# svenstaro/bvh

Measured on NVIDIA H100. Metric: traversal_Mrays_per_s, higher is better.
Workload: dtype f32

## Files before the change

bvh_b200/csrc/capi.cu:

```cuda
#include "internal.h"
#include <cstdarg>
#include <cstring>
#include <vector>
#include <new>
#include <algorithm>
#include <cctype>
#include <sched.h>

namespace bvhb200 {

static thread_local std::string g_last_error;

void set_error(const char* fmt, ...) {
    char buf[1024];
    va_list ap;
    va_start(ap, fmt);
    vsnprintf(buf, sizeof(buf), fmt, ap);
    va_end(ap);
    g_last_error = buf;
}

int dalloc(bvhgpu_ctx* ctx, void** p, size_t bytes) {
    *p = nullptr;
    if (bytes == 0) bytes = 16;
// ... 912 lines not shown
        return rc;
    }
    return BVHGPU_OK;
}
BVH_EXPORT uint64_t bvhgpu_launch_count(const bvhgpu_ctx* ctx) { return ctx ? ctx->launches : 0; }
BVH_EXPORT int bvhgpu_set_option(bvhgpu_ctx* ctx, const char* name, int64_t value) {
    if (!ctx || !name) { set_error("set_option: null argument"); return BVHGPU_ERR_INVALID; }
    if (!strcmp(name, "traverse_slots")) { ctx->traverse_slots = value; return BVHGPU_OK; }
    if (!strcmp(name, "profile")) { ctx->profile = value; return BVHGPU_OK; }
    if (!strcmp(name, "build_small")) { ctx->build_small = value; return BVHGPU_OK; }
    if (!strcmp(name, "build_gang")) { ctx->build_gang = value; return BVHGPU_OK; }
    if (!strcmp(name, "build_subtree")) { ctx->build_subtree = value; return BVHGPU_OK; }
    if (!strcmp(name, "traverse_persistent")) { ctx->traverse_persistent = value; return BVHGPU_OK; }
    if (!strcmp(name, "traverse_stream")) { ctx->traverse_stream = value; return BVHGPU_OK; }
    if (!strcmp(name, "traverse_top")) { ctx->traverse_top = value; return BVHGPU_OK; }
    if (!strcmp(name, "walk_grid")) { ctx->walk_grid = value <= 0 ? 0 : (int)value; ctx->walk_grid_forced = value > 0; return BVHGPU_OK; }
    set_error("set_option: unknown option '%s'", name);
    return BVHGPU_ERR_INVALID;
}

BVH_EXPORT int bvhgpu_get_metric(bvhgpu_ctx* ctx, const char* name, double* out) {
    if (!ctx || !name || !out) { set_error("get_metric: null argument"); return BVHGPU_ERR_INVALID; }
    cudaEvent_t* ev = nullptr;
    if (!strncmp(name, "e2e_host_us_", 12) && name[12] >= '0' && name[12] <= '7' && !name[13]) { *out = ctx->host_us[name[12] - '0']; return BVHGPU_OK; }
    if (!strcmp(name, "stream_write_value")) { *out = (double)ctx->wv_ok; return BVHGPU_OK; }
    if (!strcmp(name, "host_streamed")) { *out = (double)ctx->last_streamed; return BVHGPU_OK; }
    if (!strcmp(name, "numa_node")) { *out = (double)ctx->numa_node; return BVHGPU_OK; }
    if (!strcmp(name, "walk_ms") && ctx->have_walk) ev = ctx->ev_walk;
    else if (!strcmp(name, "build_ms") && ctx->have_build) ev = ctx->ev_build;
    if (!ev && ctx->have_e2e && !strncmp(name, "e2e_", 4)) {
// ... 317 lines not shown
```

bvh_b200/csrc/common.cuh:

```cuda
#pragma once
#include <cuda_runtime.h>
#include <stdint.h>
#include <stddef.h>
#include "../../include/bvh_b200.h"

#define BVH_INVALID 0xFFFFFFFFu

namespace bvhb200 {

template <class T> struct Traits;

struct __align__(16) DAabbF { float min[3]; uint32_t pad0; float max[3]; uint32_t pad1; };
struct __align__(16) DAabbD { double min[3]; double max[3]; };

struct __align__(16) TNodeF { float min[3]; uint32_t skip; float max[3]; uint32_t shape; };
struct __align__(16) TNodeD { double min[3]; double max[3]; uint32_t skip; uint32_t shape; uint32_t pad[2]; };

template <> struct Traits<float> {
    using Aabb = bvh_aabb3f; using Ray = bvh_ray3f; using Node = bvh_node3f; using Flat = bvh_flat3f;
    using DAabb = DAabbF; using TNode = TNodeF;
    using Key = uint32_t;
    static constexpr Key KEY_POS_INF = 0xFF800000u;
    static constexpr Key KEY_NEG_INF = 0x007FFFFFu;
    __host__ __device__ static inline float eps() { return 1.1920928955078125e-7f; }
// ... 43 lines not shown

__device__ __forceinline__ float min_t(float a, float b) { return fminf(a, b); }
__device__ __forceinline__ float max_t(float a, float b) { return fmaxf(a, b); }
__device__ __forceinline__ double min_t(double a, double b) { return fmin(a, b); }
__device__ __forceinline__ double max_t(double a, double b) { return fmax(a, b); }

__device__ __forceinline__ float mul_rn(float a, float b) { return __fmul_rn(a, b); }
__device__ __forceinline__ float add_rn(float a, float b) { return __fadd_rn(a, b); }
__device__ __forceinline__ float sub_rn(float a, float b) { return __fsub_rn(a, b); }
__device__ __forceinline__ float div_rn(float a, float b) { return __fdiv_rn(a, b); }
__device__ __forceinline__ double mul_rn(double a, double b) { return __dmul_rn(a, b); }
__device__ __forceinline__ double add_rn(double a, double b) { return __dadd_rn(a, b); }
__device__ __forceinline__ double sub_rn(double a, double b) { return __dsub_rn(a, b); }
__device__ __forceinline__ double div_rn(double a, double b) { return __ddiv_rn(a, b); }

template <class T> __device__ __forceinline__ T center1(T mn, T mx) { return add_rn(mul_rn(mn, T(0.5)), mul_rn(mx, T(0.5))); }
template <class T> __device__ __forceinline__ T surface_area(const T mn[3], const T mx[3]) {
    const T sx = sub_rn(mx[0], mn[0]), sy = sub_rn(mx[1], mn[1]), sz = sub_rn(mx[2], mn[2]);
    return mul_rn(T(2), add_rn(add_rn(mul_rn(sx, sx), mul_rn(sy, sy)), mul_rn(sz, sz)));
}

template <int D, class T>
__device__ __forceinline__ bool slab_slice(const T o[D], const T inv[D], const T mn[D], const T mx[D], T& tmin_out, T& tmax_out) {
    T l[D], r[D];
#pragma unroll
    for (int k = 0; k < D; ++k) { l[k] = mul_rn(sub_rn(mn[k], o[k]), inv[k]); r[k] = mul_rn(sub_rn(mx[k], o[k]), inv[k]); }
    bool nan = (l[0] != l[0]) | (r[0] != r[0]);
#pragma unroll
    for (int k = 1; k < D; ++k) nan = nan | (l[k] != l[k]) | (r[k] != r[k]);
    T tmin = min_t(l[0], r[0]), tmax = max_t(l[0], r[0]);
// ... 66 lines not shown
```

bvh_b200/csrc/flatten.cu:

```cuda
#include "internal.h"
#include "update.cuh"

namespace bvhb200 {

template <class T>
__global__ void __launch_bounds__(256) flat_kernel(const typename Traits<T>::Node* __restrict__ nodes,
                                                   const uint32_t* __restrict__ node_start, uint32_t n_nodes,
                                                   typename Traits<T>::Flat* __restrict__ flat, const BuildStatus* __restrict__ status) {
    using Tr = Traits<T>;
    const uint32_t i = blockIdx.x * blockDim.x + threadIdx.x;
    if (i >= n_nodes) return;
    if (status->error | status->nan_found) return;
    const uint4 meta = *reinterpret_cast<const uint4*>(nodes + i);
    const bool leaf = meta.y == BVH_INVALID;
    if (i == 0) {
        if (leaf) {
            typename Tr::Flat f;
            for (int k = 0; k < 3; ++k) { f.aabb.min[k] = Tr::inf(); f.aabb.max[k] = -Tr::inf(); }
            f.entry_index = BVH_INVALID; f.exit_index = 1; f.shape_index = meta.w;
            flat[0] = f;
        }
        return;
    }
    const uint32_t nav = (i - 1) + node_start[i];
// ... 54 lines not shown
template <class T> int build_traversal_records(Tree<T>* tree) {
    bvhgpu_ctx* ctx = tree->ctx;
    if (tree->n == 0) { tree->n_trec = 0; return BVHGPU_OK; }
    const uint32_t n_trec = tree->n == 1 ? 1u : tree->n_nodes - 1;
    if (!tree->d_tnodes) BVH_TRY(dalloc_t(ctx, &tree->d_tnodes, n_trec));
    tree->n_trec = n_trec;
    tree->top_valid = false;
    trec_kernel<T><<<(tree->n_nodes + 255) / 256, 256, 0, ctx->stream>>>(tree->d_nodes, tree->n_nodes, tree->dims == 2 && tree->d_aabb_trav ? tree->d_aabb_trav : tree->d_aabb, tree->d_tnodes, tree->d_status, tree->dims);
    ctx->launches++;
    BVH_CUDA_TRY(cudaGetLastError());
    return BVHGPU_OK;
}

constexpr uint32_t TOP_BINS = 256;
__device__ __forceinline__ uint32_t top_bin(uint32_t c) { const uint32_t k = 31 - __clz(c); return 8 * k + (((c << 3) >> k) & 7u); }
__global__ void __launch_bounds__(256) top_hist_kernel(const bvh_node3f* __restrict__ nodes, uint32_t n_nodes, uint32_t* __restrict__ hist) {
    __shared__ uint32_t sh[TOP_BINS];
    sh[threadIdx.x] = 0;
    __syncthreads();
    const uint32_t i = blockIdx.x * blockDim.x + threadIdx.x;
    if (i >= 1 && i < n_nodes) atomicAdd(sh + top_bin(nodes[nodes[i].parent].shape), 1u);
    __syncthreads();
    if (sh[threadIdx.x]) atomicAdd(hist + threadIdx.x, sh[threadIdx.x]);
}
__global__ void __launch_bounds__(32) top_choose_kernel(const uint32_t* __restrict__ hist, uint32_t budget, uint32_t* __restrict__ hdr) {
    const uint32_t l = threadIdx.x & 31u, FULL = 0xffffffffu;
    uint32_t h[8], t = 0;
#pragma unroll
    for (int k = 0; k < 8; ++k) { h[k] = hist[8 * l + k]; t += h[k]; }
    uint32_t incl = t;
#pragma unroll
    for (int o = 1; o < 32; o <<= 1) { const uint32_t v = __shfl_down_sync(FULL, incl, o); if (l + o < 32) incl += v; }
    uint32_t run = incl - t, taken = 0, total = 0;
#pragma unroll
    for (int k = 7; k >= 0; --k) { run += h[k]; if (run <= budget) { ++taken; total = run; } }
    taken = __reduce_add_sync(FULL, taken);
    total = __reduce_max_sync(FULL, total);
    if (l) return;
    uint32_t C = 2;
    if (taken == 0) C = 0xFFFFFFFFu;
    else if (taken < TOP_BINS) { const uint32_t nb = TOP_BINS - taken, k = nb >> 3, sub = nb & 7u; C = (uint32_t)((((unsigned long long)(8 + sub) << k) + 7ull) >> 3); }
    hdr[0] = total; hdr[1] = C; hdr[2] = 0; hdr[3] = 0;
}
__global__ void __launch_bounds__(256) top_flag_kernel(const bvh_node3f* __restrict__ nodes, uint32_t n_nodes, const uint32_t* __restrict__ hdr, uint32_t* __restrict__ flags) {
    const uint32_t i = blockIdx.x * blockDim.x + threadIdx.x;
    if (i > n_nodes) return;
    const uint32_t C = hdr[1];
    uint32_t f = 0;
    if (i >= 1 && i < n_nodes) f = nodes[nodes[i].parent].shape >= C ? 1u : 0u;
    flags[i] = f;
}
__global__ void __launch_bounds__(256) top_emit_kernel(const bvh_node3f* __restrict__ nodes, uint32_t n_nodes, const TNodeF* __restrict__ trec,
                                                       const uint32_t* __restrict__ flags, const uint32_t* __restrict__ pre, float4* __restrict__ top) {
    const uint32_t i = blockIdx.x * blockDim.x + threadIdx.x;
    if (i == 0 || i >= n_nodes || !flags[i]) return;
    const uint32_t n_top = reinterpret_cast<const uint32_t*>(top)[0], C = reinterpret_cast<const uint32_t*>(top)[1];
    float4* lo = top + 2;
    float4* hi = lo + n_top;
    const uint32_t k = pre[i];
    if (k >= n_top) return;
    const uint4 meta = *reinterpret_cast<const uint4*>(nodes + i);
    const bool leaf = meta.y == BVH_INVALID;
    const uint32_t cnt = leaf ? 1u : meta.w;
    const TNodeF r = trec[i - 1];
    uint32_t w3, w7;
    if (!leaf && cnt >= C) { const uint32_t end = i + 2 * cnt - 1; w3 = pre[end < n_nodes ? end : n_nodes]; w7 = 0xFFFFFFFFu; }
    else if (leaf)         { w3 = k + 1; w7 = meta.w; }
    else                   { w3 = r.skip; w7 = 0x80000000u | i; }
    lo[k] = make_float4(r.min[0], r.min[1], r.min[2], __uint_as_float(w3));
    hi[k] = make_float4(r.max[0], r.max[1], r.max[2], __uint_as_float(w7));
}
}
#include <cub/device/device_scan.cuh>
namespace bvhb200 {
int build_top_records(Tree<float>* tree, uint32_t budget) {
    bvhgpu_ctx* ctx = tree->ctx;
    cudaStream_t st = ctx->stream;
    const uint32_t nn = tree->n_nodes;
    Scratch scratch(ctx);
    uint32_t *hist = nullptr, *flags = nullptr, *pre = nullptr;
    BVH_TRY(scratch.get(&hist, TOP_BINS));
    BVH_TRY(scratch.get(&flags, (size_t)nn + 1));
    BVH_TRY(scratch.get(&pre, (size_t)nn + 1));
    if (tree->d_top && tree->top_cap < budget) { dfree(ctx, tree->d_top); tree->d_top = nullptr; }
    if (!tree->d_top) { BVH_TRY(dalloc(ctx, &tree->d_top, 32 * ((size_t)budget + 1))); tree->top_cap = budget; }
    BVH_CUDA_TRY(cudaMemsetAsync(hist, 0, TOP_BINS * sizeof(uint32_t), st));
    const unsigned g = (nn + 256) / 256;
    uint32_t* hdr = reinterpret_cast<uint32_t*>(tree->d_top);
    top_hist_kernel<<<g, 256, 0, st>>>(tree->d_nodes, nn, hist);
    top_choose_kernel<<<1, 32, 0, st>>>(hist, budget, hdr);
    top_flag_kernel<<<g, 256, 0, st>>>(tree->d_nodes, nn, hdr, flags);
    size_t tmp_bytes = 0;
    cub::DeviceScan::ExclusiveSum(nullptr, tmp_bytes, flags, pre, (int)(nn + 1), st);
    unsigned char* tmp = nullptr;
    BVH_TRY(scratch.get(&tmp, tmp_bytes));
    cub::DeviceScan::ExclusiveSum(tmp, tmp_bytes, flags, pre, (int)(nn + 1), st);
    top_emit_kernel<<<g, 256, 0, st>>>(tree->d_nodes, nn, tree->d_tnodes, flags, pre, reinterpret_cast<float4*>(tree->d_top));
    ctx->launches += 5;
    BVH_CUDA_TRY(cudaGetLastError());
    tree->top_valid = true; tree->top_budget = budget;
    return BVHGPU_OK;
}

template <class T> int build_flat(Tree<T>* tree) {
    bvhgpu_ctx* ctx = tree->ctx;
    tree->n_flat = tree->n == 0 ? 0 : (tree->n == 1 ? 1 : 3 * (size_t)tree->n - 2);
    tree->have_flat = true;
    if (tree->n == 0) return BVHGPU_OK;
    if (!tree->d_flat) BVH_TRY(dalloc_t(ctx, &tree->d_flat, tree->n_flat));
    flat_kernel<T><<<(tree->n_nodes + 255) / 256, 256, 0, ctx->stream>>>(tree->d_nodes, tree->d_node_start, tree->n_nodes, tree->d_flat, tree->d_status);
    ctx->launches++;
    BVH_CUDA_TRY(cudaGetLastError());
    return BVHGPU_OK;
}

// ... 323 lines not shown
```

bvh_b200/csrc/internal.h:

```cpp
#pragma once
#include <cuda_runtime.h>
#include <string>
#include <cstdio>
#include "common.cuh"

namespace bvhb200 {

void set_error(const char* fmt, ...);

#define BVH_CUDA_TRY(expr)                                                                          \
    do {                                                                                            \
        cudaError_t _e = (expr);                                                                    \
        if (_e != cudaSuccess) {                                                                    \
            ::bvhb200::set_error("%s failed: %s (%s:%d)", #expr, cudaGetErrorString(_e), __FILE__, __LINE__); \
            return BVHGPU_ERR_CUDA;                                                                 \
        }                                                                                           \
    } while (0)

#define BVH_TRY(expr)                  \
    do {                               \
        int _s = (expr);               \
        if (_s != BVHGPU_OK) return _s; \
    } while (0)

// ... 26 lines not shown
    int64_t profile = 0;
    cudaEvent_t ev_walk[2] = {nullptr, nullptr};
    cudaEvent_t ev_build[2] = {nullptr, nullptr};
    bool have_walk = false, have_build = false;
    cudaStream_t copy_stream = nullptr, d2h_stream = nullptr;
    cudaEvent_t ev_order = nullptr, ev_total = nullptr;
    cudaEvent_t ev_chunk[16] = {}, ev_emit[16] = {};
    cudaEvent_t ev_e2e[5] = {};
    bool have_e2e = false;
    int stream_ok = -1;
    double host_us[8] = {0, 0, 0, 0, 0, 0, 0, 0};
    uint64_t slot_budget_words = 0;
    int last_streamed = -1;
    int64_t traverse_stream = -1;
    int64_t traverse_top = -1;
    uint32_t* d_ready = nullptr;
    int wv_ok = -1;
    uint32_t* d_async_err = nullptr;
    int numa_node = -1;
};
#define BVH_MAX_CHUNKS 16u

namespace bvhb200 {

template <class T> struct Tree {
    using Tr = Traits<T>;
    bvhgpu_ctx* ctx = nullptr;
    uint32_t n = 0;
    uint32_t n_nodes = 0;
    int dims = 3;
    typename Tr::DAabb* d_aabb = nullptr;
    typename Tr::DAabb* d_aabb_trav = nullptr;
    typename Tr::Node* d_nodes = nullptr;
    uint32_t* d_node_index = nullptr;
    uint32_t* d_node_start = nullptr;
    typename Tr::TNode* d_tnodes = nullptr;
    uint32_t n_trec = 0;
    void* d_top = nullptr;
    uint32_t top_cap = 0, top_budget = 0;
    bool top_valid = false;
    uint32_t* d_arrive = nullptr;
    uint8_t* d_bad = nullptr;
    void* d_sa_base = nullptr;
    void* d_tris = nullptr;
    typename Tr::Flat* d_flat = nullptr;
    size_t n_flat = 0;
    bool have_flat = false;
    BuildStatus* d_status = nullptr;
    BuildStatus* h_status = nullptr;
    bool status_pending = false;
    int failed_status = 0;
    std::string failed_message;
    uint32_t* d_offsets = nullptr; size_t offsets_cap = 0;
    uint32_t* d_hits = nullptr;    size_t hits_cap = 0;
    size_t last_total = 0, last_nrays = 0;
// ... 26 lines not shown
template <class T> int convert_aabbs(bvhgpu_ctx* ctx, const typename Traits<T>::Aabb* in_aabbs, uint32_t n,
                                     typename Traits<T>::DAabb* out, uint32_t* d_nan_flag);

struct BuildCtl;
template <class T> struct QSlot;
template <class T> struct TreeletSession { void* params = nullptr; QSlot<T>* q = nullptr; uint32_t* qseq = nullptr; uint32_t qmask = 0; BuildCtl* ctl = nullptr; };
template <class T> int treelet_begin(bvhgpu_ctx* ctx, Tree<T>* tree, uint32_t* sorted_ids, TreeletSession<T>* S);
template <class T> int treelet_finish(bvhgpu_ctx* ctx, Tree<T>* tree, TreeletSession<T>* S);

template <class T> int rebuild_subtrees(bvhgpu_ctx* ctx, Tree<T>* tree, const uint32_t* d_roots, const uint32_t* d_n_roots, const T* cb, uint32_t* idx0, bool cb_by_root);

template <class T> int build_lbvh(bvhgpu_ctx* ctx, const typename Traits<T>::Aabb* in_aabbs, uint32_t n, Tree<T>* tree, bool treelets);

template <class T> int build_traversal_records(Tree<T>* tree);
template <class T> int build_flat(Tree<T>* tree);
int build_top_records(Tree<float>* tree, uint32_t budget);
template <class T> int sah_cost(Tree<T>* tree, double* out2);
template <class T> int refit(Tree<T>* tree);
template <class T> int optimize(Tree<T>* tree, double max_growth);
template <class T> int update_changed(Tree<T>* tree, const uint32_t* d_changed, const typename Traits<T>::Aabb* d_fresh, uint32_t m, uint32_t* d_flags);
template <class T> int update_incremental(Tree<T>* tree, const uint32_t* d_changed, uint32_t m, double max_growth);
template <class T> int update_scatter(Tree<T>* tree, const uint32_t* d_changed, const typename Traits<T>::Aabb* d_fresh, uint32_t m);
template <class T> int ensure_sa_base(Tree<T>* tree);
template <class T> int rebuild_degraded(Tree<T>* tree, const uint32_t* d_dirty, uint32_t* d_cnts );

template <class T> int add_shapes(Tree<T>* tree, typename Traits<T>::DAabb* aabb_all, uint32_t k, double max_growth);
template <class T> int remove_shapes(Tree<T>* tree, const uint32_t* d_rm, uint32_t k);
int remove_check(bvhgpu_ctx* ctx, const uint32_t* d_idx, uint32_t k, uint32_t n, uint32_t* d_rm, uint32_t* d_flags);

template <class T> int traverse_device(Tree<T>* tree, int mode, const void* d_rays, uint32_t fmt,
                                       size_t nrays, uint32_t* d_offsets, uint32_t* d_hits, size_t cap, size_t* total,
// ... 40 lines not shown
```

bvh_b200/csrc/traverse.cu:

```cuda
#include "internal.h"
#include "csr.cuh"
#include "queries.cuh"
#include <cstdlib>
#include <cstring>
#include <algorithm>
#include <chrono>

namespace bvhb200 {

static inline uint32_t pick_slots(bvhgpu_ctx* ctx, uint32_t nrays) {
    if (ctx->traverse_slots >= 0) return (uint32_t)std::min<int64_t>(ctx->traverse_slots, 64);
    uint64_t budget_words = 1ull << 30;
    if (ctx->slot_budget_words == 0) {
        size_t free_b = 0, total_b = 0;
        ctx->slot_budget_words = cudaMemGetInfo(&free_b, &total_b) == cudaSuccess ? std::max<uint64_t>((uint64_t)free_b / 16, 1) : budget_words;
    }
    budget_words = std::min<uint64_t>(budget_words, ctx->slot_budget_words);
    const uint64_t k = budget_words / std::max<uint32_t>(nrays, 1u);
    if (k < 4) return (uint32_t)k;
    uint32_t p = 4;
    while (p * 2 <= k && p < 64) p *= 2;
    return p;
}

// ... 9 lines not shown
template <> __device__ __forceinline__ double tmin2(double a, double b) { return fmin(a, b); }
template <class T> __device__ __forceinline__ T tmax2(T a, T b);
template <> __device__ __forceinline__ float tmax2(float a, float b) { return fmaxf(a, b); }
template <> __device__ __forceinline__ double tmax2(double a, double b) { return fmax(a, b); }

template <class T>
__device__ __forceinline__ bool slab_hit(const T o[3], const T inv[3], const T mn[3], const T mx[3]) {
    const T l0 = mul_rn(sub_rn(mn[0], o[0]), inv[0]), r0 = mul_rn(sub_rn(mx[0], o[0]), inv[0]);
    const T l1 = mul_rn(sub_rn(mn[1], o[1]), inv[1]), r1 = mul_rn(sub_rn(mx[1], o[1]), inv[1]);
    const T l2 = mul_rn(sub_rn(mn[2], o[2]), inv[2]), r2 = mul_rn(sub_rn(mx[2], o[2]), inv[2]);
    const bool nan = (l0 != l0) | (r0 != r0) | (l1 != l1) | (r1 != r1) | (l2 != l2) | (r2 != r2);
    const T tmin = tmax2(tmax2(tmin2(l0, r0), tmin2(l1, r1)), tmin2(l2, r2));
    const T tmax = tmin2(tmin2(tmax2(l0, r0), tmax2(l1, r1)), tmax2(l2, r2));
    const T lo = tmin > T(0) ? tmin : T(0);
    return !nan && tmax >= lo;
}

template <class T, bool FLAT, class Emit>
__device__ __forceinline__ uint32_t walk(const typename Traits<T>::TNode* __restrict__ trec, uint32_t n_rec,
                                         const typename Traits<T>::DAabb* __restrict__ aabb,
                                         const T o[3], const T inv[3], Emit emit) {
    uint32_t i = 0, visits = 0;
    while (i < n_rec) {
        T mn[3], mx[3];
        uint32_t skip, shape;
        fetch(trec + i, mn, mx, skip, shape);
        ++visits;
        if (slab_hit(o, inv, mn, mx)) {
            if (shape != BVH_INVALID) {
                bool report = true;
// ... 164 lines not shown
                if (i >= n_rec) { counts[r] = cnt; r = NONE; }
            }
            const uint32_t idle_mask = __ballot_sync(FULL, r == NONE);
            const int idle = __popc(idle_mask);
            if (idle == 32 || (idle >= REFILL && !exhausted)) break;
            if (STREAM) {
                const uint32_t pend = __ballot_sync(FULL, r != NONE && !loaded);
                if (pend && (((++rounds) & 15u) == 0u || (pend | idle_mask) == FULL)) break;
            }
        }
    }
    visits = __reduce_add_sync(FULL, visits);
    if (lane == 0 && visits) atomicAdd(visit_total, (unsigned long long)visits);
}

template <bool FLAT, bool STREAM, int VPC>
__global__ void __launch_bounds__(1024, 1) walk_top_kernel(const TNodeF* __restrict__ trec, const DAabbF* __restrict__ aabb,
                                                           uint32_t n_rec, const float4* __restrict__ top,
                                                           RaySrc<float> rays, uint32_t nrays, uint32_t* __restrict__ ticket, const uint32_t* ready,
                                                           uint32_t* __restrict__ counts, uint32_t* __restrict__ slots, uint32_t K,
                                                           unsigned long long* __restrict__ visit_total, const uint32_t* __restrict__ gate, uint32_t run_if,
                                                           uint32_t* err, unsigned long long timeout_ns, int refill) {
    extern __shared__ float4 s_top[];
    if (gate && *gate != run_if) return;
    const uint32_t n_top = reinterpret_cast<const uint32_t*>(top)[0];
    for (uint32_t k = threadIdx.x; k < 2 * n_top; k += blockDim.x) s_top[k] = top[2 + k];
    __syncthreads();
    uint32_t s_lo;
    asm volatile("mov.u32 %0, %1;" : "=r"(s_lo) : "r"((uint32_t)__cvta_generic_to_shared(s_top)));
    const uint32_t s_hi = s_lo + 16u * n_top;
    constexpr uint32_t NONE = 0xFFFFFFFFu;
    const uint32_t FULL = 0xffffffffu;
    const uint32_t lane = lane_id(), lt = lanemask_lt();
    uint32_t r = NONE, j = 0, g = 0, gend = 0, cnt = 0, visits = 0;
    bool loaded = false;
    float o[3] = {0.f, 0.f, 0.f}, inv[3] = {0.f, 0.f, 0.f};
    bool exhausted = false;
    for (;;) {
        const uint32_t need = __ballot_sync(FULL, r == NONE);
        if (need && !exhausted) {
            uint32_t base = 0;
            if (lane == 0) base = atomicAdd(ticket, (uint32_t)__popc(need));
            base = __shfl_sync(FULL, base, 0);
            if (base >= nrays) exhausted = true;
            const uint32_t mine = base + __popc(need & lt);
            if (r == NONE && mine < nrays) {
                r = mine; j = 0; cnt = 0; g = 0; gend = n_top ? 0u : n_rec;
                if (STREAM) loaded = false;
                else load_ray<float, false>(rays, mine, o, inv);
            }
        }
        if (STREAM) {
            const uint32_t pend = __ballot_sync(FULL, r != NONE && !loaded);
            if (pend) {
                const bool any_active = __ballot_sync(FULL, r != NONE && loaded) != 0u;
                const uint32_t lowest = __reduce_min_sync(FULL, (r != NONE && !loaded) ? r : NONE);
                uint32_t rd = 0, ok = 1;
                if (lane == 0) {
                    rd = *(volatile const uint32_t*)ready;
                    if (!any_active && rd <= lowest) {
                        uint32_t ns = 100;
                        const unsigned long long t0 = global_timer_ns();
                        while (rd <= lowest) {
                            if (*(volatile const uint32_t*)err != 0u) { ok = 0; break; }
                            if (global_timer_ns() - t0 > timeout_ns) { ok = 0; atomicExch(err, (uint32_t)BVHGPU_ERR_TIMEOUT); break; }
                            __nanosleep(ns);
                            if (ns < 2000) ns <<= 1;
                            rd = *(volatile const uint32_t*)ready;
                        }
                    }
                }
                rd = __shfl_sync(FULL, rd, 0);
                ok = __shfl_sync(FULL, ok, 0);
                if (!ok) {
                    exhausted = true;
                    if (r != NONE && !loaded) r = NONE;
                } else if (__ballot_sync(FULL, r != NONE && !loaded && r < rd)) {
                    __threadfence();
                    if (r != NONE && !loaded && r < rd) { load_ray<float, true>(rays, r, o, inv); loaded = true; }
                }
            }
        }
        if (__ballot_sync(FULL, r != NONE) == 0) break;
        const int leave = exhausted ? 32 : refill;
        auto visit = [&]() {
            if (r != NONE && (!STREAM || loaded)) {
                float mn[3], mx[3];
                uint32_t w3, w7;
                const bool below = g < gend;
                if (!below) {
                    float4 a, b;
                    asm("ld.shared.v4.f32 {%0,%1,%2,%3}, [%4];" : "=f"(a.x), "=f"(a.y), "=f"(a.z), "=f"(a.w) : "r"(s_lo + 16u * j));
                    asm("ld.shared.v4.f32 {%0,%1,%2,%3}, [%4];" : "=f"(b.x), "=f"(b.y), "=f"(b.z), "=f"(b.w) : "r"(s_hi + 16u * j));
                    mn[0] = a.x; mn[1] = a.y; mn[2] = a.z; w3 = __float_as_uint(a.w);
                    mx[0] = b.x; mx[1] = b.y; mx[2] = b.z; w7 = __float_as_uint(b.w);
                } else {
                    fetch(trec + g, mn, mx, w3, w7);
                }
                ++visits;
                const bool hit = slab_hit(o, inv, mn, mx);
                const bool fringe = !below && (w7 + 0x80000000u) < 0x7FFFFFFFu;
                const uint32_t cur = below ? g : j;
                const uint32_t nxt = (hit || fringe) ? cur + 1 : w3;
                if (hit && (int32_t)w7 >= 0) {
                    bool report = true;
                    if (FLAT) {
                        float smn[3], smx[3];
                        load_aabb(aabb + w7, smn, smx);
                        report = slab_hit(o, inv, smn, smx);
                    }
                    if (report) { if (cnt < K) slots[(size_t)cnt * nrays + r] = w7; ++cnt; }
                }
                j = below ? j : nxt;
                gend = below ? gend : ((hit && fringe) ? w3 : 0u);
                g = below ? nxt : (w7 & 0x7FFFFFFFu);
                if (g >= gend && j >= n_top) { counts[r] = cnt; r = NONE; }
            }
        };
        uint32_t rounds = 0;
        for (;;) {
#pragma unroll
            for (int u = 0; u < VPC; ++u) visit();
            const uint32_t idle_mask = __ballot_sync(FULL, r == NONE);
            if (__popc(idle_mask) >= leave) break;
            if (STREAM) {
                const uint32_t pend = __ballot_sync(FULL, r != NONE && !loaded);
                if (pend && (((rounds += VPC) & 15u) == 0u || (pend | idle_mask) == FULL)) break;
            }
        }
    }
    visits = __reduce_add_sync(FULL, visits);
    if (lane == 0 && visits) atomicAdd(visit_total, (unsigned long long)visits);
}

__global__ void __launch_bounds__(SCAN_THREADS) scan_local_kernel(const uint32_t* __restrict__ counts, uint32_t n,
                                                                  uint32_t* __restrict__ local, unsigned long long* __restrict__ blocksum,
                                                                  uint32_t* __restrict__ maxcount) {
// ... 397 lines not shown
                                                            RaySrc<T> rays, uint32_t nrays,
                                                            const uint32_t* __restrict__ counts, const uint32_t* __restrict__ slots, uint32_t K,
                                                            const uint32_t* __restrict__ local, const unsigned long long* __restrict__ blocksum,
                                                            const unsigned long long* __restrict__ total,
                                                            EmitDst dst, unsigned long long cap, uint32_t count,
                                                            PeerBoxes pb, const unsigned long long* __restrict__ xinfo, uint32_t* __restrict__ arrival,
                                                            uint32_t emit_blocks, uint32_t* __restrict__ offsets) {
    if (blockIdx.x < emit_blocks) emit_body<T, FLAT>(trec, n_rec, aabb, rays, nrays, counts, slots, K, local, blocksum, total, dst, cap, 0u, count, pb, xinfo, arrival, blockIdx.x, emit_blocks);
    else goffsets_body(pb, xinfo, offsets, blockIdx.x - emit_blocks, gridDim.x - emit_blocks);
}

constexpr uint32_t SUMS_TAIL = 20;
constexpr uint32_t S_TOTAL = 0, S_VISITS = 1, S_XINFO = 2, S_ERR = 12, S_TICKET = 13, S_READY = 14, S_GATE = 15, S_MAXC = 16, S_BLKDONE = 17;
constexpr unsigned long long STREAM_TIMEOUT_NS = 4ull * 1000ull * 1000ull * 1000ull;
constexpr uint32_t TOP_BUDGET = 7000;
constexpr size_t TOP_UNROLL_MAX_BYTES = (size_t)32 << 20;
template <class T> static bool launch_top(Tree<T>*, bool, RaySrc<T>, uint32_t, uint32_t*, uint32_t*, uint32_t, unsigned long long*, uint32_t*, bool) { return false; }
template <> bool launch_top<float>(Tree<float>* tree, bool flat, RaySrc<float> rays, uint32_t R, uint32_t* counts, uint32_t* slots, uint32_t K,
                                   unsigned long long* tail, uint32_t* gate, bool stream_mode) {
    bvhgpu_ctx* ctx = tree->ctx;
    if (tree->n < 2) return false;
    const uint32_t budget = ctx->traverse_top > 1 ? (uint32_t)std::min<int64_t>(std::max<int64_t>(ctx->traverse_top, 8), TOP_BUDGET) : TOP_BUDGET;
    if ((!tree->top_valid || tree->top_budget != budget) && build_top_records(tree, budget) != BVHGPU_OK) return false;
    if (!ctx->top_attr_set) {
        const int bytes = (int)(TOP_BUDGET * 32);
        auto raise = [&](const void* f) { return cudaFuncSetAttribute(f, cudaFuncAttributeMaxDynamicSharedMemorySize, bytes) == cudaSuccess; };
        if (!raise((const void*)walk_top_kernel<false, false, 1>) || !raise((const void*)walk_top_kernel<true, false, 1>) ||
            !raise((const void*)walk_top_kernel<false, true, 1>) || !raise((const void*)walk_top_kernel<true, true, 1>) ||
            !raise((const void*)walk_top_kernel<false, false, 4>) || !raise((const void*)walk_top_kernel<true, false, 4>) ||
            !raise((const void*)walk_top_kernel<false, true, 4>) || !raise((const void*)walk_top_kernel<true, true, 4>)) { cudaGetLastError(); return false; }
        ctx->top_attr_set = true;
    }
    const size_t smem = (size_t)budget * 32;
    const int grid = (int)std::min<uint64_t>((uint64_t)ctx->sm_count, ((uint64_t)R + 1023) / 1024);
    uint32_t* ticket = reinterpret_cast<uint32_t*>(tail + S_TICKET);
    uint32_t* err = reinterpret_cast<uint32_t*>(tail + S_ERR);
    const float4* top = reinterpret_cast<const float4*>(tree->d_top);
    static const int top_refill = getenv("BVHGPU_TOP_REFILL") ? std::max(1, std::min(32, atoi(getenv("BVHGPU_TOP_REFILL")))) : 8;
    const bool l2_tree = (size_t)tree->n_trec * sizeof(TNodeF) <= TOP_UNROLL_MAX_BYTES;
#define BVH_TOP_LAUNCH(F, S, V, TMO) walk_top_kernel<F, S, V><<<grid, 1024, smem, ctx->stream>>>(tree->d_tnodes, walk_aabbs(tree), tree->n_trec, top, rays, R, ticket, \
                                                                    ctx->d_ready, counts, slots, K, tail + S_VISITS, gate, 0u, err, TMO, top_refill)
#define BVH_TOP_FORMS(V) do { if (stream_mode) { if (flat) BVH_TOP_LAUNCH(true, true, V, STREAM_TIMEOUT_NS); else BVH_TOP_LAUNCH(false, true, V, STREAM_TIMEOUT_NS); } \
                              else             { if (flat) BVH_TOP_LAUNCH(true, false, V, 0ull); else BVH_TOP_LAUNCH(false, false, V, 0ull); } } while (0)
    if (l2_tree) BVH_TOP_FORMS(4); else BVH_TOP_FORMS(1);
#undef BVH_TOP_FORMS
#undef BVH_TOP_LAUNCH
    ctx->launches++;
    return true;
}

template <class T>
static int launch_pass1(Tree<T>* tree, bool flat, RaySrc<T> rays, uint32_t R, uint32_t first, uint32_t count,
                        uint32_t* counts, uint32_t* slots, uint32_t K, unsigned long long* sums, uint32_t nblk, bool stream_mode) {
    bvhgpu_ctx* ctx = tree->ctx;
    cudaStream_t st = ctx->stream;
    unsigned long long* tail = sums + nblk;
    const int64_t pmode = stream_mode ? 1 : ctx->traverse_persistent;
    uint32_t* gate = nullptr;
    if (pmode >= 2) {
// ... 549 lines not shown
```

Before: 2426.

## Add quantized compact top-level node records and a NaN-free fast slab test

Adds an optional compact top-tree format that stores 16-bit quantized child boxes (16 bytes per node) in shared memory. This fits twice as many top nodes in the same shared memory, with conservative outer and inner boxes and an exact fallback fetch when the quantized test is inconclusive. On the default path, the build now records whether the top records are NaN-free, and the walk kernel uses a cheaper slab test without NaN checks when that holds and the ray is finite. With more than one visit per round, counts writes are deferred until after the unrolled visits. The compact mode is off by default, and the whole change adds more kernel variants and register pressure.

```diff
diff --git a/bvh_b200/csrc/capi.cu b/bvh_b200/csrc/capi.cu
--- a/bvh_b200/csrc/capi.cu
+++ b/bvh_b200/csrc/capi.cu
@@ -950,6 +950,7 @@
     if (!strcmp(name, "traverse_persistent")) { ctx->traverse_persistent = value; return BVHGPU_OK; }
     if (!strcmp(name, "traverse_stream")) { ctx->traverse_stream = value; return BVHGPU_OK; }
     if (!strcmp(name, "traverse_top")) { ctx->traverse_top = value; return BVHGPU_OK; }
+    if (!strcmp(name, "traverse_top_compact")) { ctx->traverse_top_compact = value; return BVHGPU_OK; }
     if (!strcmp(name, "walk_grid")) { ctx->walk_grid = value <= 0 ? 0 : (int)value; ctx->walk_grid_forced = value > 0; return BVHGPU_OK; }
     set_error("set_option: unknown option '%s'", name);
     return BVHGPU_ERR_INVALID;
diff --git a/bvh_b200/csrc/common.cuh b/bvh_b200/csrc/common.cuh
--- a/bvh_b200/csrc/common.cuh
+++ b/bvh_b200/csrc/common.cuh
@@ -81,6 +81,21 @@
 __device__ __forceinline__ double sub_rn(double a, double b) { return __dsub_rn(a, b); }
 __device__ __forceinline__ double div_rn(double a, double b) { return __ddiv_rn(a, b); }
 
+constexpr uint32_t TOPC_EXACT = 0x80000000u, TOPC_NOHIT = 0x40000000u, TOPC_SKIP = 0x7FFFu;
+constexpr float TOPC_OUT = 8388608.0f, TOPC_IN_MN = 8388607.0f, TOPC_IN_MX = 8388609.0f;
+__device__ __forceinline__ float top_deq(uint32_t q, float bias, float cell, float org) {
+    return __fmaf_rn(__fsub_rn(__uint_as_float(0x4B000000u | q), bias), cell, org);
+}
+__device__ __forceinline__ void top_boxes(uint4 c, const float org[3], const float cell[3], float omn[3], float omx[3], float imn[3], float imx[3]) {
+    const uint32_t w[3] = {c.x, c.y, c.z};
+#pragma unroll
+    for (int k = 0; k < 3; ++k) {
+        const uint32_t a = w[k] & 0xFFFFu, b = w[k] >> 16;
+        omn[k] = top_deq(a, TOPC_OUT, cell[k], org[k]);   omx[k] = top_deq(b, TOPC_OUT, cell[k], org[k]);
+        imn[k] = top_deq(a, TOPC_IN_MN, cell[k], org[k]); imx[k] = top_deq(b, TOPC_IN_MX, cell[k], org[k]);
+    }
+}
+
 template <class T> __device__ __forceinline__ T center1(T mn, T mx) { return add_rn(mul_rn(mn, T(0.5)), mul_rn(mx, T(0.5))); }
 template <class T> __device__ __forceinline__ T surface_area(const T mn[3], const T mx[3]) {
     const T sx = sub_rn(mx[0], mn[0]), sy = sub_rn(mx[1], mn[1]), sz = sub_rn(mx[2], mn[2]);
diff --git a/bvh_b200/csrc/flatten.cu b/bvh_b200/csrc/flatten.cu
--- a/bvh_b200/csrc/flatten.cu
+++ b/bvh_b200/csrc/flatten.cu
@@ -92,16 +92,24 @@
 
 constexpr uint32_t TOP_BINS = 256;
 __device__ __forceinline__ uint32_t top_bin(uint32_t c) { const uint32_t k = 31 - __clz(c); return 8 * k + (((c << 3) >> k) & 7u); }
-__global__ void __launch_bounds__(256) top_hist_kernel(const bvh_node3f* __restrict__ nodes, uint32_t n_nodes, uint32_t* __restrict__ hist) {
+__global__ void __launch_bounds__(256) top_hist_kernel(const bvh_node3f* __restrict__ nodes, uint32_t n_nodes, const TNodeF* __restrict__ trec,
+                                                       uint32_t* __restrict__ hist) {
     __shared__ uint32_t sh[TOP_BINS];
     sh[threadIdx.x] = 0;
     __syncthreads();
     const uint32_t i = blockIdx.x * blockDim.x + threadIdx.x;
-    if (i >= 1 && i < n_nodes) atomicAdd(sh + top_bin(nodes[nodes[i].parent].shape), 1u);
+    bool nan = false;
+    if (i >= 1 && i < n_nodes) {
+        atomicAdd(sh + top_bin(nodes[nodes[i].parent].shape), 1u);
+        const TNodeF r = trec[i - 1];
+        nan = isnan(r.min[0]) | isnan(r.min[1]) | isnan(r.min[2]) | isnan(r.max[0]) | isnan(r.max[1]) | isnan(r.max[2]);
+    }
+    if (__any_sync(0xffffffffu, nan) && lane_id() == 0) atomicOr(hist + TOP_BINS, 1u);
     __syncthreads();
     if (sh[threadIdx.x]) atomicAdd(hist + threadIdx.x, sh[threadIdx.x]);
 }
-__global__ void __launch_bounds__(32) top_choose_kernel(const uint32_t* __restrict__ hist, uint32_t budget, uint32_t* __restrict__ hdr) {
+__global__ void __launch_bounds__(32) top_choose_kernel(const uint32_t* __restrict__ hist, uint32_t budget, uint32_t* __restrict__ hdr,
+                                                        const bvh_node3f* __restrict__ nodes, const TNodeF* __restrict__ trec, uint32_t compact) {
     const uint32_t l = threadIdx.x & 31u, FULL = 0xffffffffu;
     uint32_t h[8], t = 0;
 #pragma unroll
@@ -118,7 +126,44 @@
     uint32_t C = 2;
     if (taken == 0) C = 0xFFFFFFFFu;
     else if (taken < TOP_BINS) { const uint32_t nb = TOP_BINS - taken, k = nb >> 3, sub = nb & 7u; C = (uint32_t)((((unsigned long long)(8 + sub) << k) + 7ull) >> 3); }
-    hdr[0] = total; hdr[1] = C; hdr[2] = 0; hdr[3] = 0;
+    hdr[0] = total; hdr[1] = C; hdr[2] = compact; hdr[3] = hist[TOP_BINS] ? 0u : 1u;
+    if (!compact) return;
+    const TNodeF a = trec[nodes[0].child_l - 1], b = trec[nodes[0].child_r - 1];
+    float* g = reinterpret_cast<float*>(hdr + 4);
+    for (int k = 0; k < 3; ++k) {
+        const float mn = fminf(a.min[k], b.min[k]), mx = fmaxf(a.max[k], b.max[k]);
+        float cell = 0.f;
+        if (isfinite(mn) && isfinite(mx) && mn <= mx) {
+            const double ext = (double)mx - (double)mn;
+            double c = 0x1p-126;
+            while (65535.0 * c < ext && c < 0x1p111) c *= 2.0;
+            cell = (float)c;
+        }
+        g[k] = mn; g[4 + k] = cell;
+    }
+    g[3] = 0.f; g[7] = 0.f;
+}
+__device__ uint32_t top_quantize(const float org[3], const float cell[3], const float emn[3], const float emx[3], uint32_t w[3]) {
+    w[0] = w[1] = w[2] = 0u;
+    uint32_t flags = 0;
+    for (int k = 0; k < 3; ++k) {
+        const float a = emn[k], b = emx[k], c = cell[k], o = org[k];
+        if (!(c > 0.f) || !isfinite(a) || !isfinite(b) || !(a <= b)) return TOPC_EXACT | TOPC_NOHIT;
+        const double da = floor(((double)a - (double)o) / (double)c), db = ceil(((double)b - (double)o) / (double)c);
+        if (!(da >= 0.0 && da <= 65535.0 && db >= 0.0 && db <= 65535.0)) return TOPC_EXACT | TOPC_NOHIT;
+        uint32_t qa = (uint32_t)da, qb = (uint32_t)db;
+        for (int it = 0; it < 2; ++it) {
+            if (qa > 0u && top_deq(qa, TOPC_OUT, c, o) > a) --qa;
+            if (qa < 65535u && top_deq(qa + 1u, TOPC_OUT, c, o) <= a) ++qa;
+            if (qb < 65535u && top_deq(qb, TOPC_OUT, c, o) < b) ++qb;
+            if (qb > 0u && top_deq(qb - 1u, TOPC_OUT, c, o) >= b) --qb;
+        }
+        if (!(top_deq(qa, TOPC_OUT, c, o) <= a && top_deq(qb, TOPC_OUT, c, o) >= b)) return TOPC_EXACT | TOPC_NOHIT;
+        const float ia = top_deq(qa, TOPC_IN_MN, c, o), ib = top_deq(qb, TOPC_IN_MX, c, o);
+        if (!(ia >= a && ib <= b && ia <= ib)) flags = TOPC_NOHIT;
+        w[k] = qa | (qb << 16);
+    }
+    return flags;
 }
 __global__ void __launch_bounds__(256) top_flag_kernel(const bvh_node3f* __restrict__ nodes, uint32_t n_nodes, const uint32_t* __restrict__ hdr, uint32_t* __restrict__ flags) {
     const uint32_t i = blockIdx.x * blockDim.x + threadIdx.x;
@@ -128,13 +173,12 @@
     if (i >= 1 && i < n_nodes) f = nodes[nodes[i].parent].shape >= C ? 1u : 0u;
     flags[i] = f;
 }
+template <bool COMPACT>
 __global__ void __launch_bounds__(256) top_emit_kernel(const bvh_node3f* __restrict__ nodes, uint32_t n_nodes, const TNodeF* __restrict__ trec,
                                                        const uint32_t* __restrict__ flags, const uint32_t* __restrict__ pre, float4* __restrict__ top) {
     const uint32_t i = blockIdx.x * blockDim.x + threadIdx.x;
     if (i == 0 || i >= n_nodes || !flags[i]) return;
     const uint32_t n_top = reinterpret_cast<const uint32_t*>(top)[0], C = reinterpret_cast<const uint32_t*>(top)[1];
-    float4* lo = top + 2;
-    float4* hi = lo + n_top;
     const uint32_t k = pre[i];
     if (k >= n_top) return;
     const uint4 meta = *reinterpret_cast<const uint4*>(nodes + i);
@@ -145,38 +189,55 @@
     if (!leaf && cnt >= C) { const uint32_t end = i + 2 * cnt - 1; w3 = pre[end < n_nodes ? end : n_nodes]; w7 = 0xFFFFFFFFu; }
     else if (leaf)         { w3 = k + 1; w7 = meta.w; }
     else                   { w3 = r.skip; w7 = 0x80000000u | i; }
-    lo[k] = make_float4(r.min[0], r.min[1], r.min[2], __uint_as_float(w3));
-    hi[k] = make_float4(r.max[0], r.max[1], r.max[2], __uint_as_float(w7));
+    if constexpr (COMPACT) {
+        TNodeF x = r;
+        x.skip = w3; x.shape = w7;
+        reinterpret_cast<TNodeF*>(top + 4)[k] = x;
+        const float4 org = top[1], cell = top[2];
+        const float o3[3] = {org.x, org.y, org.z}, c3[3] = {cell.x, cell.y, cell.z};
+        uint32_t q[3];
+        uint32_t link = top_quantize(o3, c3, r.min, r.max, q);
+        const bool inner = w7 == 0xFFFFFFFFu;
+        if (!inner) link |= TOPC_NOHIT;
+        link |= inner ? w3 : k + 1;
+        reinterpret_cast<uint4*>(top + 4 + 2 * n_top)[k] = make_uint4(q[0], q[1], q[2], link);
+    } else {
+        float4* lo = top + 2;
+        float4* hi = lo + n_top;
+        lo[k] = make_float4(r.min[0], r.min[1], r.min[2], __uint_as_float(w3));
+        hi[k] = make_float4(r.max[0], r.max[1], r.max[2], __uint_as_float(w7));
+    }
 }
 }
 #include <cub/device/device_scan.cuh>
 namespace bvhb200 {
-int build_top_records(Tree<float>* tree, uint32_t budget) {
+int build_top_records(Tree<float>* tree, uint32_t budget, bool compact) {
     bvhgpu_ctx* ctx = tree->ctx;
     cudaStream_t st = ctx->stream;
     const uint32_t nn = tree->n_nodes;
     Scratch scratch(ctx);
     uint32_t *hist = nullptr, *flags = nullptr, *pre = nullptr;
-    BVH_TRY(scratch.get(&hist, TOP_BINS));
+    BVH_TRY(scratch.get(&hist, TOP_BINS + 1));
     BVH_TRY(scratch.get(&flags, (size_t)nn + 1));
     BVH_TRY(scratch.get(&pre, (size_t)nn + 1));
     if (tree->d_top && tree->top_cap < budget) { dfree(ctx, tree->d_top); tree->d_top = nullptr; }
-    if (!tree->d_top) { BVH_TRY(dalloc(ctx, &tree->d_top, 32 * ((size_t)budget + 1))); tree->top_cap = budget; }
-    BVH_CUDA_TRY(cudaMemsetAsync(hist, 0, TOP_BINS * sizeof(uint32_t), st));
+    if (!tree->d_top) { BVH_TRY(dalloc(ctx, &tree->d_top, 64 + 48 * (size_t)budget)); tree->top_cap = budget; }
+    BVH_CUDA_TRY(cudaMemsetAsync(hist, 0, (TOP_BINS + 1) * sizeof(uint32_t), st));
     const unsigned g = (nn + 256) / 256;
     uint32_t* hdr = reinterpret_cast<uint32_t*>(tree->d_top);
-    top_hist_kernel<<<g, 256, 0, st>>>(tree->d_nodes, nn, hist);
-    top_choose_kernel<<<1, 32, 0, st>>>(hist, budget, hdr);
+    top_hist_kernel<<<g, 256, 0, st>>>(tree->d_nodes, nn, tree->d_tnodes, hist);
+    top_choose_kernel<<<1, 32, 0, st>>>(hist, budget, hdr, tree->d_nodes, tree->d_tnodes, compact ? 1u : 0u);
     top_flag_kernel<<<g, 256, 0, st>>>(tree->d_nodes, nn, hdr, flags);
     size_t tmp_bytes = 0;
     cub::DeviceScan::ExclusiveSum(nullptr, tmp_bytes, flags, pre, (int)(nn + 1), st);
     unsigned char* tmp = nullptr;
     BVH_TRY(scratch.get(&tmp, tmp_bytes));
     cub::DeviceScan::ExclusiveSum(tmp, tmp_bytes, flags, pre, (int)(nn + 1), st);
-    top_emit_kernel<<<g, 256, 0, st>>>(tree->d_nodes, nn, tree->d_tnodes, flags, pre, reinterpret_cast<float4*>(tree->d_top));
+    if (compact) top_emit_kernel<true><<<g, 256, 0, st>>>(tree->d_nodes, nn, tree->d_tnodes, flags, pre, reinterpret_cast<float4*>(tree->d_top));
+    else         top_emit_kernel<false><<<g, 256, 0, st>>>(tree->d_nodes, nn, tree->d_tnodes, flags, pre, reinterpret_cast<float4*>(tree->d_top));
     ctx->launches += 5;
     BVH_CUDA_TRY(cudaGetLastError());
-    tree->top_valid = true; tree->top_budget = budget;
+    tree->top_valid = true; tree->top_budget = budget; tree->top_compact = compact;
     return BVHGPU_OK;
 }
 
diff --git a/bvh_b200/csrc/internal.h b/bvh_b200/csrc/internal.h
--- a/bvh_b200/csrc/internal.h
+++ b/bvh_b200/csrc/internal.h
@@ -64,6 +64,7 @@
     int last_streamed = -1;
     int64_t traverse_stream = -1;
     int64_t traverse_top = -1;
+    int64_t traverse_top_compact = -1;
     uint32_t* d_ready = nullptr;
     int wv_ok = -1;
     uint32_t* d_async_err = nullptr;
@@ -88,7 +89,7 @@
     uint32_t n_trec = 0;
     void* d_top = nullptr;
     uint32_t top_cap = 0, top_budget = 0;
-    bool top_valid = false;
+    bool top_valid = false, top_compact = false;
     uint32_t* d_arrive = nullptr;
     uint8_t* d_bad = nullptr;
     void* d_sa_base = nullptr;
@@ -145,7 +146,7 @@
 
 template <class T> int build_traversal_records(Tree<T>* tree);
 template <class T> int build_flat(Tree<T>* tree);
-int build_top_records(Tree<float>* tree, uint32_t budget);
+int build_top_records(Tree<float>* tree, uint32_t budget, bool compact);
 template <class T> int sah_cost(Tree<T>* tree, double* out2);
 template <class T> int refit(Tree<T>* tree);
 template <class T> int optimize(Tree<T>* tree, double max_growth);
diff --git a/bvh_b200/csrc/traverse.cu b/bvh_b200/csrc/traverse.cu
--- a/bvh_b200/csrc/traverse.cu
+++ b/bvh_b200/csrc/traverse.cu
@@ -5,6 +5,7 @@
 #include <cstring>
 #include <algorithm>
 #include <chrono>
+#include <type_traits>
 
 namespace bvhb200 {
 
@@ -47,6 +48,26 @@
     const T tmax = tmin2(tmin2(tmax2(l0, r0), tmax2(l1, r1)), tmax2(l2, r2));
     const T lo = tmin > T(0) ? tmin : T(0);
     return !nan && tmax >= lo;
+}
+
+__device__ __forceinline__ bool slab_hit_finite(const float o[3], const float inv[3], const float mn[3], const float mx[3]) {
+    const float l0 = mul_rn(sub_rn(mn[0], o[0]), inv[0]), r0 = mul_rn(sub_rn(mx[0], o[0]), inv[0]);
+    const float l1 = mul_rn(sub_rn(mn[1], o[1]), inv[1]), r1 = mul_rn(sub_rn(mx[1], o[1]), inv[1]);
+    const float l2 = mul_rn(sub_rn(mn[2], o[2]), inv[2]), r2 = mul_rn(sub_rn(mx[2], o[2]), inv[2]);
+    const float tmin = fmaxf(fmaxf(fminf(l0, r0), fminf(l1, r1)), fminf(l2, r2));
+    const float tmax = fminf(fminf(fmaxf(l0, r0), fmaxf(l1, r1)), fmaxf(l2, r2));
+    return tmax >= (tmin > 0.f ? tmin : 0.f);
+}
+
+__device__ __forceinline__ bool slab_hit_top(const float o[3], const float inv[3], const float mn[3], const float mx[3], bool fast) {
+    const float l0 = mul_rn(sub_rn(mn[0], o[0]), inv[0]), r0 = mul_rn(sub_rn(mx[0], o[0]), inv[0]);
+    const float l1 = mul_rn(sub_rn(mn[1], o[1]), inv[1]), r1 = mul_rn(sub_rn(mx[1], o[1]), inv[1]);
+    const float l2 = mul_rn(sub_rn(mn[2], o[2]), inv[2]), r2 = mul_rn(sub_rn(mx[2], o[2]), inv[2]);
+    const float tmin = fmaxf(fmaxf(fminf(l0, r0), fminf(l1, r1)), fminf(l2, r2));
+    const float tmax = fminf(fminf(fmaxf(l0, r0), fmaxf(l1, r1)), fmaxf(l2, r2));
+    bool hit = tmax >= (tmin > 0.f ? tmin : 0.f);
+    if (!fast) hit = hit && !((l0 != l0) | (r0 != r0) | (l1 != l1) | (r1 != r1) | (l2 != l2) | (r2 != r2));
+    return hit;
 }
 
 template <class T, bool FLAT, class Emit>
@@ -241,7 +262,14 @@
     if (lane == 0 && visits) atomicAdd(visit_total, (unsigned long long)visits);
 }
 
-template <bool FLAT, bool STREAM, int VPC>
+__device__ __forceinline__ bool ray_finite(const float o[3], const float inv[3]) {
+    bool ok = true;
+#pragma unroll
+    for (int k = 0; k < 3; ++k) ok = ok && isfinite(o[k]) && isfinite(inv[k]) && inv[k] != 0.f;
+    return ok;
+}
+
+template <bool FLAT, bool STREAM, int VPC, bool COMPACT>
 __global__ void __launch_bounds__(1024, 1) walk_top_kernel(const TNodeF* __restrict__ trec, const DAabbF* __restrict__ aabb,
                                                            uint32_t n_rec, const float4* __restrict__ top,
                                                            RaySrc<float> rays, uint32_t nrays, uint32_t* __restrict__ ticket, const uint32_t* ready,
@@ -251,15 +279,25 @@
     extern __shared__ float4 s_top[];
     if (gate && *gate != run_if) return;
     const uint32_t n_top = reinterpret_cast<const uint32_t*>(top)[0];
-    for (uint32_t k = threadIdx.x; k < 2 * n_top; k += blockDim.x) s_top[k] = top[2 + k];
+    const float4* src = COMPACT ? top + 4 + 2 * n_top : top + 2;
+    for (uint32_t k = threadIdx.x; k < (COMPACT ? n_top : 2 * n_top); k += blockDim.x) s_top[k] = src[k];
     __syncthreads();
     uint32_t s_lo;
     asm volatile("mov.u32 %0, %1;" : "=r"(s_lo) : "r"((uint32_t)__cvta_generic_to_shared(s_top)));
-    const uint32_t s_hi = s_lo + 16u * n_top;
+    uint32_t s_hi = s_lo + 16u * n_top;
+    if (VPC > 1) asm volatile("mov.u32 %0, %1;" : "=r"(s_hi) : "r"(s_lo + 16u * n_top));
+    const bool nan_free = reinterpret_cast<const uint32_t*>(top)[3] != 0u;
+    const TNodeF* xtop = reinterpret_cast<const TNodeF*>(top + 4);
+    float gorg[3] = {0.f, 0.f, 0.f}, gcell[3] = {0.f, 0.f, 0.f};
+    if (COMPACT) {
+        const float4 a = top[1], b = top[2];
+        gorg[0] = a.x; gorg[1] = a.y; gorg[2] = a.z; gcell[0] = b.x; gcell[1] = b.y; gcell[2] = b.z;
+    }
+    bool ray_ok = false;
     constexpr uint32_t NONE = 0xFFFFFFFFu;
     const uint32_t FULL = 0xffffffffu;
     const uint32_t lane = lane_id(), lt = lanemask_lt();
-    uint32_t r = NONE, j = 0, g = 0, gend = 0, cnt = 0, visits = 0;
+    uint32_t r = NONE, j = 0, g = 0, gend = 0, cnt = 0, visits = 0, done = NONE;
     bool loaded = false;
     float o[3] = {0.f, 0.f, 0.f}, inv[3] = {0.f, 0.f, 0.f};
     bool exhausted = false;
@@ -274,7 +312,7 @@
             if (r == NONE && mine < nrays) {
                 r = mine; j = 0; cnt = 0; g = 0; gend = n_top ? 0u : n_rec;
                 if (STREAM) loaded = false;
-                else load_ray<float, false>(rays, mine, o, inv);
+                else { load_ray<float, false>(rays, mine, o, inv); ray_ok = ray_finite(o, inv); }
             }
         }
         if (STREAM) {
@@ -304,28 +342,50 @@
                     if (r != NONE && !loaded) r = NONE;
                 } else if (__ballot_sync(FULL, r != NONE && !loaded && r < rd)) {
                     __threadfence();
-                    if (r != NONE && !loaded && r < rd) { load_ray<float, true>(rays, r, o, inv); loaded = true; }
+                    if (r != NONE && !loaded && r < rd) { load_ray<float, true>(rays, r, o, inv); loaded = true; ray_ok = ray_finite(o, inv); }
                 }
             }
         }
         if (__ballot_sync(FULL, r != NONE) == 0) break;
         const int leave = exhausted ? 32 : refill;
-        auto visit = [&]() {
+        const bool wfast = VPC > 1 && nan_free && __all_sync(FULL, ray_ok || r == NONE || (STREAM && !loaded));
+        auto visit = [&](auto fast_c) {
+            constexpr bool FAST = decltype(fast_c)::value;
             if (r != NONE && (!STREAM || loaded)) {
                 float mn[3], mx[3];
                 uint32_t w3, w7;
                 const bool below = g < gend;
-                if (!below) {
-                    float4 a, b;
-                    asm("ld.shared.v4.f32 {%0,%1,%2,%3}, [%4];" : "=f"(a.x), "=f"(a.y), "=f"(a.z), "=f"(a.w) : "r"(s_lo + 16u * j));
-                    asm("ld.shared.v4.f32 {%0,%1,%2,%3}, [%4];" : "=f"(b.x), "=f"(b.y), "=f"(b.z), "=f"(b.w) : "r"(s_hi + 16u * j));
-                    mn[0] = a.x; mn[1] = a.y; mn[2] = a.z; w3 = __float_as_uint(a.w);
-                    mx[0] = b.x; mx[1] = b.y; mx[2] = b.z; w7 = __float_as_uint(b.w);
+                bool hit;
+                if (COMPACT) {
+                    bool exact = below;
+                    hit = false; w3 = 0u; w7 = 0xFFFFFFFFu;
+                    if (!below) {
+                        uint4 c;
+                        asm("ld.shared.v4.u32 {%0,%1,%2,%3}, [%4];" : "=r"(c.x), "=r"(c.y), "=r"(c.z), "=r"(c.w) : "r"(s_lo + 16u * j));
+                        float omn[3], omx[3], imn[3], imx[3];
+                        top_boxes(c, gorg, gcell, omn, omx, imn, imx);
+                        const bool dmiss = ray_ok & !(c.w & TOPC_EXACT) & !slab_hit_finite(o, inv, omn, omx);
+                        const bool dhit = ray_ok & !(c.w & TOPC_NOHIT) & slab_hit_finite(o, inv, imn, imx);
+                        exact = !(dmiss || dhit);
+                        hit = dhit; w3 = c.w & TOPC_SKIP;
+                    }
+                    if (exact) {
+                        fetch(below ? trec + g : xtop + j, mn, mx, w3, w7);
+                        hit = slab_hit_top(o, inv, mn, mx, FAST);
+                    }
                 } else {
-                    fetch(trec + g, mn, mx, w3, w7);
+                    if (!below) {
+                        float4 a, b;
+                        asm("ld.shared.v4.f32 {%0,%1,%2,%3}, [%4];" : "=f"(a.x), "=f"(a.y), "=f"(a.z), "=f"(a.w) : "r"(s_lo + 16u * j));
+                        asm("ld.shared.v4.f32 {%0,%1,%2,%3}, [%4];" : "=f"(b.x), "=f"(b.y), "=f"(b.z), "=f"(b.w) : "r"(s_hi + 16u * j));
+                        mn[0] = a.x; mn[1] = a.y; mn[2] = a.z; w3 = __float_as_uint(a.w);
+                        mx[0] = b.x; mx[1] = b.y; mx[2] = b.z; w7 = __float_as_uint(b.w);
+                    } else {
+                        fetch(trec + g, mn, mx, w3, w7);
+                    }
+                    hit = slab_hit_top(o, inv, mn, mx, FAST);
                 }
                 ++visits;
-                const bool hit = slab_hit(o, inv, mn, mx);
                 const bool fringe = !below && (w7 + 0x80000000u) < 0x7FFFFFFFu;
                 const uint32_t cur = below ? g : j;
                 const uint32_t nxt = (hit || fringe) ? cur + 1 : w3;
@@ -341,13 +401,22 @@
                 j = below ? j : nxt;
                 gend = below ? gend : ((hit && fringe) ? w3 : 0u);
                 g = below ? nxt : (w7 & 0x7FFFFFFFu);
-                if (g >= gend && j >= n_top) { counts[r] = cnt; r = NONE; }
+                if (g >= gend && j >= n_top) {
+                    if (VPC > 1) done = r; else counts[r] = cnt;
+                    r = NONE;
+                }
             }
         };
         uint32_t rounds = 0;
         for (;;) {
-#pragma unroll
-            for (int u = 0; u < VPC; ++u) visit();
+            if (wfast) {
+#pragma unroll
+                for (int u = 0; u < VPC; ++u) visit(std::true_type{});
+            } else {
+#pragma unroll
+                for (int u = 0; u < VPC; ++u) visit(std::false_type{});
+            }
+            if (VPC > 1 && done != NONE) { counts[done] = cnt; done = NONE; }
             const uint32_t idle_mask = __ballot_sync(FULL, r == NONE);
             if (__popc(idle_mask) >= leave) break;
             if (STREAM) {
@@ -775,35 +844,46 @@
 constexpr uint32_t S_TOTAL = 0, S_VISITS = 1, S_XINFO = 2, S_ERR = 12, S_TICKET = 13, S_READY = 14, S_GATE = 15, S_MAXC = 16, S_BLKDONE = 17;
 constexpr unsigned long long STREAM_TIMEOUT_NS = 4ull * 1000ull * 1000ull * 1000ull;
 constexpr uint32_t TOP_BUDGET = 7000;
+constexpr uint32_t TOP_BUDGET_COMPACT = 14000;
 constexpr size_t TOP_UNROLL_MAX_BYTES = (size_t)32 << 20;
 template <class T> static bool launch_top(Tree<T>*, bool, RaySrc<T>, uint32_t, uint32_t*, uint32_t*, uint32_t, unsigned long long*, uint32_t*, bool) { return false; }
 template <> bool launch_top<float>(Tree<float>* tree, bool flat, RaySrc<float> rays, uint32_t R, uint32_t* counts, uint32_t* slots, uint32_t K,
                                    unsigned long long* tail, uint32_t* gate, bool stream_mode) {
     bvhgpu_ctx* ctx = tree->ctx;
     if (tree->n < 2) return false;
-    const uint32_t budget = ctx->traverse_top > 1 ? (uint32_t)std::min<int64_t>(std::max<int64_t>(ctx->traverse_top, 8), TOP_BUDGET) : TOP_BUDGET;
-    if ((!tree->top_valid || tree->top_budget != budget) && build_top_records(tree, budget) != BVHGPU_OK) return false;
+    const bool compact = ctx->traverse_top_compact == 1;
+    const uint32_t cap = compact ? TOP_BUDGET_COMPACT : TOP_BUDGET, esize = compact ? 16u : 32u;
+    const uint32_t budget = ctx->traverse_top > 1 ? (uint32_t)std::min<int64_t>(std::max<int64_t>(ctx->traverse_top, 8), cap) : cap;
+    if ((!tree->top_valid || tree->top_budget != budget || tree->top_compact != compact) && build_top_records(tree, budget, compact) != BVHGPU_OK) return false;
     if (!ctx->top_attr_set) {
         const int bytes = (int)(TOP_BUDGET * 32);
+        static_assert(TOP_BUDGET * 32 == TOP_BUDGET_COMPACT * 16, "both forms use the same shared memory");
         auto raise = [&](const void* f) { return cudaFuncSetAttribute(f, cudaFuncAttributeMaxDynamicSharedMemorySize, bytes) == cudaSuccess; };
-        if (!raise((const void*)walk_top_kernel<false, false, 1>) || !raise((const void*)walk_top_kernel<true, false, 1>) ||
-            !raise((const void*)walk_top_kernel<false, true, 1>) || !raise((const void*)walk_top_kernel<true, true, 1>) ||
-            !raise((const void*)walk_top_kernel<false, false, 4>) || !raise((const void*)walk_top_kernel<true, false, 4>) ||
-            !raise((const void*)walk_top_kernel<false, true, 4>) || !raise((const void*)walk_top_kernel<true, true, 4>)) { cudaGetLastError(); return false; }
+        const void* forms[] = {
+            (const void*)walk_top_kernel<false, false, 1, false>, (const void*)walk_top_kernel<true, false, 1, false>,
+            (const void*)walk_top_kernel<false, true, 1, false>,  (const void*)walk_top_kernel<true, true, 1, false>,
+            (const void*)walk_top_kernel<false, false, 4, false>, (const void*)walk_top_kernel<true, false, 4, false>,
+            (const void*)walk_top_kernel<false, true, 4, false>,  (const void*)walk_top_kernel<true, true, 4, false>,
+            (const void*)walk_top_kernel<false, false, 1, true>,  (const void*)walk_top_kernel<true, false, 1, true>,
+            (const void*)walk_top_kernel<false, true, 1, true>,   (const void*)walk_top_kernel<true, true, 1, true>,
+            (const void*)walk_top_kernel<false, false, 4, true>,  (const void*)walk_top_kernel<true, false, 4, true>,
+            (const void*)walk_top_kernel<false, true, 4, true>,   (const void*)walk_top_kernel<true, true, 4, true>};
+        for (const void* f : forms) if (!raise(f)) { cudaGetLastError(); return false; }
         ctx->top_attr_set = true;
     }
-    const size_t smem = (size_t)budget * 32;
+    const size_t smem = (size_t)budget * esize;
     const int grid = (int)std::min<uint64_t>((uint64_t)ctx->sm_count, ((uint64_t)R + 1023) / 1024);
     uint32_t* ticket = reinterpret_cast<uint32_t*>(tail + S_TICKET);
     uint32_t* err = reinterpret_cast<uint32_t*>(tail + S_ERR);
     const float4* top = reinterpret_cast<const float4*>(tree->d_top);
     static const int top_refill = getenv("BVHGPU_TOP_REFILL") ? std::max(1, std::min(32, atoi(getenv("BVHGPU_TOP_REFILL")))) : 8;
     const bool l2_tree = (size_t)tree->n_trec * sizeof(TNodeF) <= TOP_UNROLL_MAX_BYTES;
-#define BVH_TOP_LAUNCH(F, S, V, TMO) walk_top_kernel<F, S, V><<<grid, 1024, smem, ctx->stream>>>(tree->d_tnodes, walk_aabbs(tree), tree->n_trec, top, rays, R, ticket, \
-                                                                    ctx->d_ready, counts, slots, K, tail + S_VISITS, gate, 0u, err, TMO, top_refill)
-#define BVH_TOP_FORMS(V) do { if (stream_mode) { if (flat) BVH_TOP_LAUNCH(true, true, V, STREAM_TIMEOUT_NS); else BVH_TOP_LAUNCH(false, true, V, STREAM_TIMEOUT_NS); } \
-                              else             { if (flat) BVH_TOP_LAUNCH(true, false, V, 0ull); else BVH_TOP_LAUNCH(false, false, V, 0ull); } } while (0)
-    if (l2_tree) BVH_TOP_FORMS(4); else BVH_TOP_FORMS(1);
+#define BVH_TOP_LAUNCH(F, S, V, C, TMO) walk_top_kernel<F, S, V, C><<<grid, 1024, smem, ctx->stream>>>(tree->d_tnodes, walk_aabbs(tree), tree->n_trec, top, rays, R, \
+                                                                    ticket, ctx->d_ready, counts, slots, K, tail + S_VISITS, gate, 0u, err, TMO, top_refill)
+#define BVH_TOP_FORMS(V, C) do { if (stream_mode) { if (flat) BVH_TOP_LAUNCH(true, true, V, C, STREAM_TIMEOUT_NS); else BVH_TOP_LAUNCH(false, true, V, C, STREAM_TIMEOUT_NS); } \
+                                 else             { if (flat) BVH_TOP_LAUNCH(true, false, V, C, 0ull); else BVH_TOP_LAUNCH(false, false, V, C, 0ull); } } while (0)
+    if (compact) { if (l2_tree) BVH_TOP_FORMS(4, true); else BVH_TOP_FORMS(1, true); }
+    else         { if (l2_tree) BVH_TOP_FORMS(4, false); else BVH_TOP_FORMS(1, false); }
 #undef BVH_TOP_FORMS
 #undef BVH_TOP_LAUNCH
     ctx->launches++;
```

After: 2516, median of 6. 3.7% higher.
